# MrSwordFish/rvel-mcmc

Measured on AMD Instinct MI355X. Metric: walker-logL evals/sec (2-planet, 100 obs, 4096 walkers); ESS/sec, higher is better.
Workload: dtype f64

## Files before the change

### include/rvmcmc.h

```cpp
#ifndef RVMCMC_H
#define RVMCMC_H

#include <stddef.h>
#include <stdint.h>

#ifdef __cplusplus
extern "C" {
#endif

#define RVM_ABI_VERSION 12

#define RVM_STATUS_OK 0
#define RVM_STATUS_PRIOR 1
#define RVM_STATUS_ENCOUNTER 2
#define RVM_STATUS_NONFINITE 3
#define RVM_STATUS_UNRESOLVED 4
#define RVM_STATUS_SKIPPED 5

#define RVM_MAX_PLANETS 4
#define RVM_MAX_LEVELS 6
#define RVM_MAX_EPOCHS_PER_DIRECTION 1700
#define RVM_SMALA_MAX_PARAMS 20
#define RVM_RESOLVE_MAX_LIMIT 12

// ... 8 lines not shown
    double resolve_tol;
    int32_t resolve_max;
} rvm_config;

typedef struct rvm_plan rvm_plan;

int rvm_plan_create(const rvm_config* cfg, const double* t, const double* rv, const double* sigma, int32_t n_obs,
                    int32_t max_walkers, rvm_plan** out);
void rvm_plan_destroy(rvm_plan* plan);
int rvm_plan_info(const rvm_plan* plan, int32_t* steps_fwd, int32_t* steps_bwd, int32_t* epochs_fwd,
                  int32_t* epochs_bwd);
#define RVM_EXT_MAX_BYTES (4ull << 30)
int rvm_plan_extension(const rvm_plan* plan, int32_t* ext_mult);
int rvm_plan_set_verify_eccentricity(rvm_plan* plan, double e);

int rvm_plan_set_certain_reject(rvm_plan* plan, int32_t on);

int rvm_plan_faults(rvm_plan* plan, int32_t reset, int64_t* handoff_timeouts, int64_t* nonfinite,
                    int64_t* unresolved, int64_t* refined, int64_t* truncated, void* stream);
#define RVM_N_COUNTERS 7
int rvm_plan_counters(rvm_plan* plan, int32_t reset, int64_t* out, int32_t n, void* stream);
int rvm_plan_hedge_stats(rvm_plan* plan, int32_t reset, int64_t* hedged, int64_t* replayed, int64_t* missed,
                         void* stream);
int rvm_plan_time_kernels(rvm_plan* plan, int32_t max_launches);
int rvm_plan_kernel_times(rvm_plan* plan, float* logl_ms, float* refine_ms, int32_t max, int32_t* n_out);
int rvm_plan_set_handoff_timeout(rvm_plan* plan, double seconds);

int rvm_logl_batch(const rvm_plan* plan, int32_t n_walkers, const double* params, double hill_factor,
                   double* logl_out, int32_t* status_out, double* rv_out, void* stream);


int rvm_stretch_propose(int32_t n_params, int32_t n_s0, int64_t s0_begin, const double* x, int32_t n_s1,
                        const double* c, double a, uint64_t seed, uint64_t iteration, uint32_t half,
                        const double* draws, double* q_out, double* z_out, void* stream);
int rvm_stretch_accept(int32_t n_params, int32_t n_s0, int64_t s0_begin, double* x, double* lnp, const double* q,
                       const double* lnp_new, const double* z, uint64_t seed, uint64_t iteration, uint32_t half,
                       const double* draws, int32_t* accepted, void* stream);

#define RVM_MAX_PARAM_ROWS (7 * RVM_MAX_PLANETS)
typedef struct rvm_param_map {
    int32_t n_rows;
    int32_t src[RVM_MAX_PARAM_ROWS];
    double base[RVM_MAX_PARAM_ROWS];
} rvm_param_map;

int rvm_stretch_half_step(const rvm_plan* plan, const rvm_param_map* map, int32_t n_params, int32_t n_s0,
// ... 106 lines not shown
```

### rvel-mcmc_amd/csrc/host_sanitize.cpp

```cpp
#include <cmath>
#include <cstdio>
#include <cstring>
#include <vector>

#include "../../include/rvmcmc.h"

int main() {
    int fails = 0;
    auto expect = [&](bool ok, const char* what) {
        if (!ok) {
            std::fprintf(stderr, "FAIL %s\n", what);
            fails++;
        }
    };
    expect(rvm_abi_version() == RVM_ABI_VERSION, "abi version");
    rvm_config cfg{};
    cfg.n_planets = 2;
    cfg.dt = 0.65;
    cfg.n_levels = 4;
    cfg.npoints_norm = 100.0;
    const int mult[4] = {4, 5, 6, 7};
    std::memcpy(cfg.level_mult, mult, sizeof(mult));
    cfg.period_hint = 5.2;
    std::vector<double> t, rv, sg;
// ... 1 lines not shown
        t.push_back(i % 2 ? -0.6 * i : 0.55 * (100 - i));
        rv.push_back(1e-4 * std::sin(i));
        sg.push_back(1.5e-4);
    }
    t[7] = t[9];
    rvm_plan* plan = nullptr;
    const int rc = rvm_plan_create(&cfg, t.data(), rv.data(), sg.data(), (int)t.size(), 4096, &plan);
    expect(rc == 0 || (rc < 0 && plan == nullptr), "plan_create valid input");
    if (rc == 0) rvm_plan_destroy(plan);
    rvm_config bad = cfg;
    bad.n_levels = 0;
    expect(rvm_plan_create(&bad, t.data(), rv.data(), sg.data(), (int)t.size(), 64, &plan) < 0, "n_levels 0");
    bad = cfg;
    bad.level_mult[1] = 4;
    expect(rvm_plan_create(&bad, t.data(), rv.data(), sg.data(), (int)t.size(), 64, &plan) < 0, "dup multipliers");
    bad = cfg;
    bad.dt = -1.0;
    expect(rvm_plan_create(&bad, t.data(), rv.data(), sg.data(), (int)t.size(), 64, &plan) < 0, "negative dt");
    std::vector<double> tn = t;
    tn[3] = NAN;
    expect(rvm_plan_create(&cfg, tn.data(), rv.data(), sg.data(), (int)t.size(), 64, &plan) < 0, "nan epoch");
    expect(std::strlen(rvm_last_error()) > 0, "last_error");
    expect(rvm_logl_batch(nullptr, 1, nullptr, 1.0, nullptr, nullptr, nullptr, nullptr) < 0, "logl null plan");
    rvm_param_map pm{};
    expect(rvm_stretch_half_step(nullptr, &pm, 10, 1, 0, nullptr, nullptr, nullptr, 1, nullptr, 2.0, 0, 0, 0, 1.0,
                                 nullptr, nullptr, nullptr, nullptr) < 0,
           "half_step null plan");
    expect(rvm_stretch_propose(0, 1, 0, nullptr, 1, nullptr, 2.0, 0, 0, 0, nullptr, nullptr, nullptr, nullptr) < 0,
           "propose bad");
    double d1 = 0.5;
    int32_t i1 = 0;
    expect(rvm_pt_stretch_propose(10, 0, 1, &d1, &d1, 2.0, 0, 0, 0, nullptr, &d1, &d1, nullptr) < 0, "pt n_temps 0");
    expect(rvm_pt_stretch_propose(10, 2, 1, &d1, &d1, 1.0, 0, 0, 0, nullptr, &d1, &d1, nullptr) < 0, "pt a = 1");
    expect(rvm_pt_stretch_propose(10, 1 << 16, 1 << 16, &d1, &d1, 2.0, 0, 0, 0, nullptr, &d1, &d1, nullptr) < 0,
           "pt int32 overflow");
    expect(rvm_pt_stretch_accept(10, 2, 1, nullptr, &d1, &d1, &d1, &d1, &d1, 0, 0, 0, nullptr, &i1, nullptr) < 0,
           "pt null betas");
    expect(rvm_pt_stretch_accept(10, 2, 1, &d1, &d1, &d1, &d1, &d1, &d1, 0, 0, 2, nullptr, &i1, nullptr) < 0,
           "pt half 2");
    expect(rvm_pt_swap(10, 2, 0, &d1, &d1, &d1, &d1, &d1, 0, 0, nullptr, &i1, nullptr) < 0, "pt n_half 0");
    expect(rvm_pt_swap(10, 1 << 15, 1 << 15, &d1, &d1, &d1, &d1, &d1, 0, 0, nullptr, &i1, nullptr) < 0,
           "pt swap int32 overflow");
    expect(rvm_pt_swap(10, 1, 4, nullptr, nullptr, nullptr, nullptr, nullptr, 0, 0, nullptr, nullptr, nullptr) == 0,
           "pt swap of one temperature");
    int64_t l1 = 0;
    expect(rvm_pt_ladder_update(3, 1, &i1, &d1, &d1, -1.0, &d1, &l1, &d1, &l1, nullptr, &d1, nullptr) < 0,
// ... 20 lines not shown
```

### rvel-mcmc_amd/csrc/rvm_abi.hip

```cpp
#include <hip/hip_runtime.h>

#include <algorithm>
#include <cmath>
#include <cstdio>
#include <cstdlib>
#include <cstring>
#include <string>
#include <vector>

#include "rvm_internal.h"

#ifndef RVM_EAGER_DEFAULT
#define RVM_EAGER_DEFAULT true
#endif
#ifndef RVM_EAGER_PASSES_DEFAULT
#define RVM_EAGER_PASSES_DEFAULT 1
#endif

namespace rvm {
hipError_t launch_logl(const DevPlan& P, int W, const double* params, double hill_factor, unsigned long long* slots,
                       double* logl, int32_t* status, double* rv_out, const StretchArgs& sa, hipStream_t stream,
                       int* dry_blocks);
hipError_t launch_refine(const DevPlan& P, int W, const double* params, double hill_factor, double* logl,
                         int32_t* status, double* rv_out, const StretchArgs& sa, int eager, int hedge,
// ... 492 lines not shown
        P.rq_tf = reinterpret_cast<unsigned long long*>(base + b_x + b_xf + b_t);
        P.rq_c = reinterpret_cast<double*>(base + b_x + b_xf + b_t + b_tf);
        P.rq_w = reinterpret_cast<int32_t*>(base + b_x + b_xf + b_t + b_tf + b_c);
        P.rq_n = reinterpret_cast<int32_t*>(base + b_x + b_xf + b_t + b_tf + b_c + b_w);
        P.gen_dev = reinterpret_cast<unsigned long long*>(base + b_x + b_xf + b_t + b_tf + b_c + b_w + 32);
        P.depth_w = reinterpret_cast<unsigned long long*>(base + b_x + b_xf + b_t + b_tf + b_c + b_w + 64 + b_m);
        P.rq_mark = reinterpret_cast<int32_t*>(base + b_x + b_xf + b_t + b_tf + b_c + b_w + 64);
        const unsigned long long gen1 = 1;
        if (hipMemcpy(P.gen_dev, &gen1, sizeof(gen1), hipMemcpyHostToDevice) != hipSuccess) {
            (void)hipGetLastError();
            rvm_plan_destroy(plan);
            return fail(-3, "rvm_plan_create: initialising the launch generation failed");
        }
        P.rq_cap = max_walkers;
        P.rq_xgroups = (int32_t)xg;
        if (const char* sp = getenv("RVM_REFINE_SPLIT"))
            if (sp[0] == '0') P.rq_x = nullptr;
        if (n_teams < 2) P.rq_t = nullptr;
        if (const char* th = getenv("RVM_TEAMS_HINT"))
            if (th[0] == '0') P.depth_w = nullptr;
        P.n_teams = (int32_t)nt;
    }
    P.hedge_groups = 0;
    P.hrv = nullptr;
    P.hsum = nullptr;
    P.hslot = nullptr;
    P.htab = nullptr;
    P.hw = nullptr;
    {
        const char* eg = getenv("RVM_EAGER");
        const bool eager_on = eg ? eg[0] == '1' : RVM_EAGER_DEFAULT;
        const int emw = std::min<int>(max_walkers, rvm::RVM_EAGER_MAX);
        const char* hg = getenv("RVM_HEDGE");
        int hgroups = hg && hg[0] == '0' ? 0 : rvm::RVM_HEDGE_GROUPS_MAX;
        if (const char* hn = getenv("RVM_HEDGE_GROUPS"))
            hgroups = std::min(hgroups, std::max(0, std::min(atoi(hn), (int)rvm::RVM_HEDGE_GROUPS_MAX)));
        if (hgroups > 0 && P.rmax >= 2 && P.rvp != nullptr && P.gen_dev != nullptr && cfg->n_levels <= 4 &&
            max_walkers >= rvm::RVM_EAGER_MIN && P.n_cu >= 4) {
            const size_t hs = rvm::RVM_HEDGE_STRIDE;
            const size_t n_rv = 2 * (size_t)P.lvx_emax * hs, n_sum = 6 * hs, n_slot = 2 * hs;
            const size_t n_all = n_rv + n_sum + n_slot + (size_t)max_walkers + rvm::RVM_HW_WORDS;
            if (hipMalloc(&plan->hmem, n_all * sizeof(double)) == hipSuccess &&
                hipMemset(plan->hmem, 0, n_all * sizeof(double)) == hipSuccess && hipDeviceSynchronize() == hipSuccess) {
                P.hrv = reinterpret_cast<double*>(plan->hmem);
                P.hsum = P.hrv + n_rv;
                P.hslot = reinterpret_cast<unsigned long long*>(P.hsum + n_sum);
                P.htab = P.hslot + n_slot;
                P.hw = P.htab + max_walkers;
                P.hedge_groups = hgroups;
            } else {
                (void)hipGetLastError();
                if (plan->hmem) (void)hipFree(plan->hmem);
                plan->hmem = nullptr;
            }
        }
        const bool eager_plan = P.rmax >= 2 && P.rvp != nullptr && P.gen_dev != nullptr && cfg->n_levels <= 4 &&
                                eager_on && max_walkers >= rvm::RVM_EAGER_MIN;
        if (!eager_plan && P.hedge_groups > 0) {
            if (hipStreamCreateWithFlags(&plan->side, hipStreamNonBlocking) != hipSuccess ||
                hipEventCreateWithFlags(&plan->ev_fork, hipEventDisableTiming) != hipSuccess ||
                hipEventCreateWithFlags(&plan->ev_join, hipEventDisableTiming) != hipSuccess) {
                (void)hipGetLastError();
                if (plan->ev_fork) (void)hipEventDestroy(plan->ev_fork);
                if (plan->ev_join) (void)hipEventDestroy(plan->ev_join);
                if (plan->side) (void)hipStreamDestroy(plan->side);
                plan->side = nullptr;
                plan->ev_fork = plan->ev_join = nullptr;
                P.hedge_groups = 0;
            }
        }
        if (eager_plan) {
            const size_t plane = (size_t)P.lvx_emax * P.lvx_stride;
// ... 97 lines not shown
        if (plan->lvmem) e = hipMemsetAsync(plan->lvmem, 0xFF, plan->lv_bytes, st);
        if (e == hipSuccess) e = hipMemsetAsync(plan->dev.counters, 0, sizeof(h), st);
        if (e == hipSuccess) e = hipStreamSynchronize(st);
        if (e != hipSuccess) return hip_fail(e, "rvm_plan_counters: reset");
    }
    return 0;
}

int rvm_plan_hedge_stats(rvm_plan* plan, int32_t reset, int64_t* hedged, int64_t* replayed, int64_t* missed,
                         void* stream) {
    if (!plan) return fail(-1, "rvm_plan_hedge_stats: null plan");
    unsigned long long h[3] = {};
    if (plan->dev.hw != nullptr) {
        hipStream_t st = (hipStream_t)stream;
        unsigned long long* d = plan->dev.hw + rvm::RVM_HW_STATS;
        hipError_t e = hipMemcpyAsync(h, d, sizeof(h), hipMemcpyDeviceToHost, st);
        if (e == hipSuccess && reset) e = hipMemsetAsync(d, 0, sizeof(h), st);
        if (e == hipSuccess) e = hipStreamSynchronize(st);
        if (e != hipSuccess) return hip_fail(e, "rvm_plan_hedge_stats");
    }
    if (hedged) *hedged = (int64_t)h[0];
    if (replayed) *replayed = (int64_t)h[1];
    if (missed) *missed = (int64_t)h[2];
    return 0;
}

int rvm_plan_faults(rvm_plan* plan, int32_t reset, int64_t* handoff_timeouts, int64_t* nonfinite,
                    int64_t* unresolved, int64_t* refined, int64_t* truncated, void* stream) {
    if (!plan) return fail(-1, "rvm_plan_faults: null plan");
    int64_t c[RVM_N_COUNTERS] = {};
    const int rc = rvm_plan_counters(plan, reset, c, RVM_N_COUNTERS, stream);
    if (rc != 0) return rc;
    if (handoff_timeouts) *handoff_timeouts = c[0];
    if (nonfinite) *nonfinite = c[1];
    if (unresolved) *unresolved = c[2];
    if (refined) *refined = c[3];
    if (truncated) *truncated = c[4];
    return 0;
}

int rvm_plan_time_kernels(rvm_plan* plan, int32_t max_launches) {
    if (!plan) return fail(-1, "rvm_plan_time_kernels: null plan");
    if (max_launches < 0 || max_launches > 4096) return fail(-1, "rvm_plan_time_kernels: max_launches out of range");
    while ((int32_t)plan->tev.size() < 3 * max_launches) {
        hipEvent_t ev;
        const hipError_t e = hipEventCreate(&ev);
// ... 527 lines not shown
```

### rvel-mcmc_amd/csrc/rvm_internal.h

```cpp
#pragma once
#include <stdint.h>

#include "../../include/rvmcmc.h"

namespace rvm {

constexpr int RVM_LS_RING = 64;
constexpr int RVM_LC_RING = 16;
constexpr int RVM_LC_RING_BYTES = 24 * 1024;
constexpr int RVM_LDS_PER_CU = 160 * 1024;
constexpr int RVM_INIT_DOUBLES = 8 * 64;
constexpr double RVM_EXT_ACCEPT = 1.0;
constexpr double RVM_CUT_EST_FACTOR = 100.0;
constexpr double RVM_FLOOR_BOUND = 4.0;
constexpr double RVM_CUT_ECC_FACTOR = 0.6712;
constexpr double RVM_CUT_GUARD_K = 10.0;
constexpr int RVM_CX_MIN_WALKERS = 32;
constexpr int RVM_EAGER_MAX = 512;
constexpr int RVM_EAGER_MIN = 32;
constexpr int RVM_EFLAG_WORDS = 8;
constexpr int RVM_TEAMS_MAX = 4;
constexpr int RVM_TEAMS_DEFAULT = 4;
constexpr int RVM_DEPTH_WINDOW = 8;
constexpr int RVM_HEDGE_GROUPS_MAX = 8;
constexpr int RVM_HEDGE_STRIDE = 512;
constexpr int RVM_HEDGE_CAND = RVM_HEDGE_STRIDE + 64;
constexpr int RVM_HEDGE_MAX_W = 12288;
constexpr int RVM_HW_STATS = 2 + 2 * RVM_HEDGE_GROUPS_MAX;
constexpr int RVM_HW_WORDS = RVM_HW_STATS + 3 + 3;

struct DirSched {
    int32_t n_epochs;
    int32_t n_steps;
    int32_t split0, pre0, split1, pre1;
    const int32_t* seg_n;
    const double* seg_h1;
    const double* obs_rv;
    const double* obs_s2;
    const int32_t* obs_idx;
};

struct DevPlan {
    int32_t n_planets;
    int32_t n_levels;
    int32_t mult[RVM_MAX_LEVELS];
    int32_t nt[RVM_MAX_LEVELS];
    int32_t spec[RVM_MAX_LEVELS];
    int32_t late_mult;
    int32_t lc_ring;
    double inv_mult[RVM_MAX_LEVELS];
    double lw[RVM_MAX_LEVELS];
    double lw3[RVM_MAX_LEVELS];
// ... 11 lines not shown
    double cut_guard_k;
    int32_t lvx_emax, lvx_stride;
    int32_t* rq_n;
    int32_t* rq_w;
    double* rq_c;
    int32_t rq_cap;
    int32_t* rq_mark;
    int32_t skip_variants;
    unsigned long long* rq_x;
    unsigned long long* rq_xf;
    int32_t rq_xgroups;
    unsigned long long* rq_t;
    unsigned long long* rq_tf;
    double* rvp2;
    int32_t n_teams;
    unsigned long long* depth_w;
    double* rve;
    double* esum;
    unsigned long long* eflag;
    int32_t eager_max;
    int32_t eager_passes;
    int32_t eager_split;
    int32_t hedge_groups;
    double* hrv;
    double* hsum;
    unsigned long long* hslot;
    unsigned long long* htab;
    unsigned long long* hw;
    unsigned long long* gen_dev;
    unsigned long long* counters;
    unsigned long long spin_ticks;
    double npoints;
    int32_t n_obs;
    int32_t inclined;
    int32_t n_cu;
    double* lv_rv;
    int32_t* lv_enc;
    int32_t lv_emax, lv_stride;
    DirSched fwd, bwd;
};

struct StretchArgs {
    const double* c;
    double* x;
    double* x_aos;
    double* lnp;
// ... 71 lines not shown
```

### rvel-mcmc_amd/csrc/rvm_refine_impl.h

```cpp
#pragma once
#include <hip/hip_runtime.h>
#include <math.h>

#pragma clang fp contract(on)

#include "rvm_walker.h"

#ifndef RVM_REFINE_GUESS
#define RVM_REFINE_GUESS 0
#endif
#ifndef RVM_REFINE_RELAXED_COUNT
#define RVM_REFINE_RELAXED_COUNT 0
#endif

namespace rvm {

#ifdef RVM_PROFILE
#define RVM_RPROF_SLOTS 20
#define RVM_RPROF_MAX_WAVES 4096
static __device__ unsigned long long rvm_rprof[RVM_RPROF_MAX_WAVES * RVM_RPROF_SLOTS];
#define RPROF_T(v) const unsigned long long v = __builtin_readcyclecounter()
#define RPROF_RT(v) const unsigned long long v = __builtin_amdgcn_s_memrealtime()
#else
#define RPROF_T(v)
#define RPROF_RT(v)
#endif

__device__ __forceinline__ bool claim_item(gu64* w, unsigned long long gen, unsigned long long code) {
    unsigned long long v = __hip_atomic_load(w, __ATOMIC_RELAXED, __HIP_MEMORY_SCOPE_AGENT);
    for (;;) {
        if ((v >> 8) == gen) return false;
        unsigned long long expect = v;
        if (__hip_atomic_compare_exchange_strong(w, &expect, (gen << 8) | code, __ATOMIC_RELAXED, __ATOMIC_RELAXED,
                                                 __HIP_MEMORY_SCOPE_AGENT))
            return true;
        v = expect;
    }
}

__device__ __forceinline__ unsigned long long pass_ticks(const DevPlan& P, int rf) {
    const unsigned long long t = P.spin_ticks << (rf < RVM_RESOLVE_MAX_LIMIT ? rf : RVM_RESOLVE_MAX_LIMIT);
    constexpr unsigned long long cap = 6000000000ull;
    return t < cap ? t : (P.spin_ticks > cap ? P.spin_ticks : cap);
}

struct DirState {
    int open;
    double chi, lb, pest, best, bchi;
};

template <int NP, bool D3, int NW>
__global__ __launch_bounds__(NW * 64) void refine_kernel(const DevPlan P, const int W, const double* __restrict__ params,
                                                     const double hill_factor, double* __restrict__ rv_out,
                                                     double* __restrict__ logl_out, int32_t* __restrict__ status_out,
                                                     const StretchArgs sa, const int eager, const int hedge) {
    constexpr int L = LanesPerWalker<NP>::value;
    constexpr int WPB = 64 / L;
    constexpr int PR = D3 ? 7 : 5;
    constexpr int R = PR * NP;
    const int wv = threadIdx.x >> 6;
    const int lane = threadIdx.x & 63;
    const int slot = lane / L;
    const int pl_idx = lane % L;
    const int nl = P.n_levels;
    RPROF_T(pt_entry);
    RPROF_RT(prt_entry);
#ifdef RVM_PROFILE
    unsigned long long p_seg = 0, p_epo = 0, p_steps = 0, p_wait = 0, p_pass = 0;
    int p_lvl = -1;
#endif

    __shared__ int s_n[3];
    __shared__ unsigned long long s_gen;
    __shared__ int s_depth;
    if (threadIdx.x == 0) {
        for (int i = 0; i < 3; i++) s_n[i] = __hip_atomic_load(P.rq_n + i, __ATOMIC_RELAXED, __HIP_MEMORY_SCOPE_AGENT);
        const unsigned long long g0 = __hip_atomic_load(P.gen_dev, __ATOMIC_RELAXED, __HIP_MEMORY_SCOPE_AGENT);
        s_gen = g0;
// ... 35 lines not shown
            gu64* hw = (gu64*)P.hw;
            if (__hip_atomic_fetch_add(hw + 1, 1ull, __ATOMIC_RELAXED, __HIP_MEMORY_SCOPE_AGENT) + 1 == gridDim.x) {
                __hip_atomic_store(hw + 1, 0ull, __ATOMIC_RELAXED, __HIP_MEMORY_SCOPE_AGENT);
                __hip_atomic_store(hw, (gen << 8) | 1ull, __ATOMIC_RELAXED, __HIP_MEMORY_SCOPE_AGENT);
            }
        }
    };
    const bool split = !eager && P.rq_x != nullptr && gq0 <= P.rq_xgroups && ((int)gridDim.x & 1) == 0 &&
                       ntask_split <= gfit;
    int nteam = 0;
    if (split && P.rq_t != nullptr && P.rvp != nullptr && P.rvp2 != nullptr && rv_out == nullptr &&
        ng <= P.rq_xgroups) {
        nteam = P.n_teams < P.rmax ? P.n_teams : P.rmax;
        if (nteam > (depth_hint > 2 ? depth_hint : 2)) nteam = depth_hint > 2 ? depth_hint : 2;
        while (nteam >= 2 && nteam * ntask_split > gfit) nteam--;
    }
    const bool team = nteam >= 2;
    const int ntask_team = nteam * ntask_split;
    const int ngw = (W + WPB - 1) / WPB;
    const bool esplit = eager && P.eager_split && P.rq_x != nullptr && ngw <= P.rq_xgroups &&
                        ((int)gridDim.x & 1) == 0 && 2 * ngw <= (int)gridDim.x;
    const int ntask = eager ? (esplit ? 2 * ngw : ngw) : (team ? ntask_team : (split ? ntask_split : ng));
    if ((int)blockIdx.x >= ntask) {
        leave();
        return;
    }

    extern __shared__ double s_sched[];
    __shared__ double s_rv[2][2][RVM_MAX_LEVELS][64];
    __shared__ int s_enc[2][RVM_MAX_LEVELS][64];
    __shared__ double s_init[8][64];
    __shared__ double s_chi[2][64], s_lb[2][64];
    __shared__ double s_pest[2][64], s_best[2][64], s_bchi[2][64];
    __shared__ int s_open[2][64];
    __shared__ int s_live[64];
    __shared__ int s_stw[64];
    __shared__ double s_lpw[64];
    __shared__ double s_acc[3][64];
    __shared__ int s_dmode[64];
    __shared__ unsigned long long s_mask[2];
    __shared__ int s_xfault;
    __shared__ double s_tc2[2][64], s_te2[2][64];
    __shared__ int s_ter[2][64];
    __shared__ int s_cancel[2];
    __shared__ int s_eitems[64], s_eli[64], s_eany;
    __shared__ int s_emask;
// ... 965 lines not shown
    const int pl_idx = lane % L;
    const int nl = P.n_levels;
    const int g = blockIdx.x >> 1, dd = blockIdx.x & 1;
    const DirSched& SR = dd ? P.bwd : P.fwd;
    const int Er = SR.n_epochs;
    extern __shared__ unsigned long long s_key[];
    __shared__ double s_rv[2][RVM_MAX_LEVELS][64];
    __shared__ int s_enc[RVM_MAX_LEVELS][64];
    __shared__ int s_cnt[2][256];
    __shared__ unsigned long long s_ck[RVM_HEDGE_CAND];
    __shared__ int s_ci[RVM_HEDGE_CAND];
    __shared__ int s_sel[64];
    __shared__ int s_cancel[2];
    __shared__ unsigned long long s_gen, s_pref;
    __shared__ int s_need;
#ifdef RVM_PROFILE
    const unsigned long long prt_entry = __builtin_amdgcn_s_memrealtime();
#endif
    gu64* hw = (gu64*)P.hw;
    if (tid == 0) s_gen = __hip_atomic_load(P.gen_dev, __ATOMIC_RELAXED, __HIP_MEMORY_SCOPE_AGENT);
    __syncthreads();
    const unsigned long long gen = s_gen;
    const unsigned long long ctag = (gen << 8) | 1ull;
    if (tid == 0) s_cancel[0] = __hip_atomic_load(hw, __ATOMIC_RELAXED, __HIP_MEMORY_SCOPE_AGENT) == ctag;
    __syncthreads();
    if (s_cancel[0]) return;
    const unsigned long long kbad = ~0ull;
    for (int i = tid; i < RVM_HEDGE_CAND; i += 256) {
        s_ck[i] = kbad;
        s_ci[i] = 0;
    }
    for (int i = tid; i < W; i += 256) {
        int kind = 0, wk = i, jst = 0, jp = 0;
        double zst = 0.0, zp = 0.0;
        stretch_slot(sa, i, kind, wk, zst, jst, zp, jp);
        double sc = INFINITY;
        bool ok = true;
#pragma unroll
        for (int p = 0; p < NP; p++) {
            const double m = walker_param(true, nullptr, W, wk, sa, PR * p + 0, zst, jst, kind, zp, jp);
            const double a = walker_param(true, nullptr, W, wk, sa, PR * p + 1, zst, jst, kind, zp, jp);
            const double h = walker_param(true, nullptr, W, wk, sa, PR * p + 2, zst, jst, kind, zp, jp);
            const double k = walker_param(true, nullptr, W, wk, sa, PR * p + 3, zst, jst, kind, zp, jp);
            const double e = sqrt(h * h + k * k);
            ok = ok && a > 0.02 && m > 5e-6 && e < 1.0;
            sc = fmin(sc, a * (1.0 - e) / cbrt(1.0 + m));
        }
        ok = ok && isfinite(sc) && sc > 0.0;
        s_key[i] = ok ? (unsigned long long)__double_as_longlong(sc) : kbad;
// ... 135 lines not shown
    KickPrep<NP> kq0{};
    if (work && Er > 0) kq0 = kick_prep<NP, L, D3>(s, 1.875);
    constexpr int rf = 2;
    const int m_r = P.mult[k_u] << rf;
    const int nt_r = P.nt[k_u];
    const bool late = P.late_mult > 0 && m_r >= P.late_mult;
    const double sc = ldexp(P.inv_mult[k_u], -rf);
    const bool cmb = work && k == 0 && lane < cnt;
    const int hx = g * WPB + (cmb ? lane : 0);
    gu64* rvo = (gu64*)(P.hrv + (size_t)dd * P.lvx_emax * RVM_HEDGE_STRIDE + hx);
    double c2 = 0.0, e2 = 0.0;
    bool cancelled = false;
#ifdef RVM_PROFILE
    const unsigned long long prt_loop0 = __builtin_amdgcn_s_memrealtime();
#endif
    for (int e = 0; e < Er; e++) {
        const int ns = __builtin_amdgcn_readfirstlane(work ? SR.seg_n[e] * m_r : 0);
        if (ns > 0)
            (void)segment_gated_c<D3, NP, L, RVM_REFINE_GUESS>(s, kq0, SR.seg_h1[e] * sc, ns, nt_r, hw, nullptr, ctag, late);
        if (work) {
            const double v0 = star_vx<NP, L>(s);
            if (pl_idx == 0) s_rv[e & 1][k_u][slot] = v0;
        }
        if (wv == 0 && lane == 0)
            s_cancel[e & 1] = __hip_atomic_load(hw, __ATOMIC_RELAXED, __HIP_MEMORY_SCOPE_AGENT) == ctag;
        __syncthreads();
        if (s_cancel[e & 1]) {
            cancelled = true;
            break;
        }
        if (cmb) {
            double rvx = 0.0, rv3 = 0.0;
            for (int q = 0; q < nl; q++) rvx += P.lw[q] * s_rv[e & 1][q][lane];
            for (int q = 1; q < nl; q++) rv3 += P.lw3[q] * s_rv[e & 1][q][lane];
            const double ob = SR.obs_rv[e], s2 = SR.obs_s2[e];
            const double r = rvx - ob;
            c2 += (r * r) / s2;
            e2 += fabs((rvx - rv3) * (r + (rv3 - ob))) / s2;
            __hip_atomic_store(rvo + (size_t)e * RVM_HEDGE_STRIDE, (unsigned long long)__double_as_longlong(rvx),
                               __ATOMIC_RELAXED, __HIP_MEMORY_SCOPE_AGENT);
        }
    }
#ifdef RVM_PROFILE
    if (lane == 0 && RVM_RPROF_MAX_WAVES / 2 + (size_t)blockIdx.x * 8 + wv < RVM_RPROF_MAX_WAVES) {
        unsigned long long* o = rvm_rprof + (RVM_RPROF_MAX_WAVES / 2 + (size_t)blockIdx.x * 8 + wv) * RVM_RPROF_SLOTS;
        o[0] = prt_entry;
        o[1] = prt_loop0;
        o[2] = __builtin_amdgcn_s_memrealtime();
        o[3] = o[2];
        o[9] = (unsigned long long)blockIdx.x | (1ull << 29) | ((unsigned long long)(cancelled ? 1 : 0) << 30);
        o[10] = cancelled ? 0 : 1;
        o[11] = (unsigned long long)(unsigned)__builtin_amdgcn_s_getreg((31 << 11) | 4);
    }
#endif
    if (cancelled) return;
    if (work && pl_idx == 0) s_enc[k_u][slot] = (int)(((s.encm >> lane) & kick_enc_bits<NP>()) != 0);
    __syncthreads();
    if (wv == 0) {
        if (__builtin_amdgcn_readfirstlane((int)(__hip_atomic_load(hw, __ATOMIC_RELAXED, __HIP_MEMORY_SCOPE_AGENT) == ctag)))
            return;
        if (cmb) {
            int er = 0;
            for (int q = 0; q < nl; q++) er |= s_enc[q][lane];
            gu64* es = (gu64*)(P.hsum + (size_t)dd * 3 * RVM_HEDGE_STRIDE + hx);
            auto bits = [](double v) { return (unsigned long long)__double_as_longlong(v); };
            __hip_atomic_store(es, bits(c2), __ATOMIC_RELAXED, __HIP_MEMORY_SCOPE_AGENT);
            __hip_atomic_store(es + RVM_HEDGE_STRIDE, bits(e2), __ATOMIC_RELAXED, __HIP_MEMORY_SCOPE_AGENT);
            __hip_atomic_store(es + 2 * RVM_HEDGE_STRIDE, bits((double)er), __ATOMIC_RELAXED, __HIP_MEMORY_SCOPE_AGENT);
        }
        asm volatile("s_waitcnt vmcnt(0)" ::: "memory");
        if (lane == 0)
            __hip_atomic_store(hw + 2 + 2 * g + dd, (gen << 8) | 2ull, __ATOMIC_RELAXED, __HIP_MEMORY_SCOPE_AGENT);
    }
}

template <int NPV, bool D3V>
static size_t hedge_budget() {
    static size_t budget[64] = {};
    static bool known[64] = {};
    int dev = 0;
    if (hipGetDevice(&dev) != hipSuccess || dev < 0 || dev >= 64) {
        (void)hipGetLastError();
        return 0;
// ... 52 lines not shown
        }
        (void)hipGetLastError();
        budget[dev] = b;
    }
    return budget[dev];
}

template <int NPV, bool D3V>
static hipError_t launch_refine_t(const DevPlan& P, int W, const double* params, double hill_factor, double* logl,
                                  int32_t* status, double* rv_out, const StretchArgs& sa, int eager, int hedge,
                                  hipStream_t stream) {
    constexpr int wpb = 64 / LanesPerWalker<NPV>::value;
    const int emax = P.fwd.n_epochs > P.bwd.n_epochs ? P.fwd.n_epochs : P.bwd.n_epochs;
    const size_t smem = (size_t)emax * 8 * sizeof(double);
    static const bool w4_env = [] {
        const char* e = getenv("RVM_REFINE_W4");
        return !(e && e[0] == '0');
    }();
    const bool w4 = P.n_levels <= 4 && w4_env;
    if (smem > (w4 ? refine_budget<NPV, D3V, 4>() : refine_budget<NPV, D3V, 8>())) return hipErrorInvalidConfiguration;
    const int groups = (W + wpb - 1) / wpb + 2;
    int nb = std::max(2, std::min(P.n_cu > 0 ? P.n_cu : 256, 2 * groups));
    nb &= ~1;
    if (w4)
        refine_kernel<NPV, D3V, 4><<<dim3(nb), dim3(256), smem, stream>>>(P, W, params, hill_factor, rv_out, logl, status,
                                                                          sa, eager, hedge);
    else
        refine_kernel<NPV, D3V, 8><<<dim3(nb), dim3(512), smem, stream>>>(P, W, params, hill_factor, rv_out, logl, status,
                                                                          sa, eager, hedge);
    return hipGetLastError();
}

template <int NPV, bool D3V>
static hipError_t prepare_refine_t(const DevPlan& P) {
    const int emax = P.fwd.n_epochs > P.bwd.n_epochs ? P.fwd.n_epochs : P.bwd.n_epochs;
    const size_t smem = (size_t)emax * 8 * sizeof(double);
    const size_t b = std::min(refine_budget<NPV, D3V, 4>(), refine_budget<NPV, D3V, 8>());
    if (P.hedge_groups > 0) (void)hedge_budget<NPV, D3V>();
    return smem <= b ? hipSuccess : hipErrorInvalidConfiguration;
}

#define RVM_REFINE_NP_API(N)                                                                                     \
    hipError_t launch_refine_np##N(const DevPlan& P, int W, const double* params, double hill_factor, double* logl, \
                                   int32_t* status, double* rv_out, const StretchArgs& sa, int eager, int hedge, \
                                   hipStream_t stream);                                                          \
    int hedge_groups_np##N(const DevPlan& P, int W, int logl_blocks);                                           \
    hipError_t launch_hedge_np##N(const DevPlan& P, int W, double hill_factor, const StretchArgs& sa, int ngrp, \
                                  hipStream_t stream);                                                           \
    hipError_t launch_eager_np##N(const DevPlan& P, int W, const double* params, double hill_factor,            \
                                  hipStream_t stream);                                                           \
    hipError_t prepare_refine_np##N(const DevPlan& P);
RVM_REFINE_NP_API(1)
RVM_REFINE_NP_API(2)
RVM_REFINE_NP_API(3)
RVM_REFINE_NP_API(4)
#undef RVM_REFINE_NP_API

}
```

### rvel-mcmc_amd/rvmcmc/_lib.py

```python
from __future__ import annotations

import ctypes as C
import os

_HERE = os.path.dirname(os.path.abspath(__file__))
LIB_PATH = os.environ.get("RVM_LIB_PATH") or os.path.join(_HERE, "librvmcmc.so")

RVM_STATUS_OK = 0
RVM_STATUS_PRIOR = 1
RVM_STATUS_ENCOUNTER = 2
RVM_STATUS_NONFINITE = 3
RVM_STATUS_UNRESOLVED = 4
RVM_STATUS_SKIPPED = 5
RVM_MAX_PLANETS = 4
RVM_MAX_LEVELS = 6
RVM_N_COUNTERS = 7
ABI_VERSION = 12


class RvmConfig(C.Structure):
    _fields_ = [
        ("n_planets", C.c_int32),
        ("dt", C.c_double),
        ("n_levels", C.c_int32),
# ... 46 lines not shown
                                         C.c_double, C.c_double, C.c_double, C.POINTER(SmalaCache), _dp]),
    "rvm_smala_center_accept": (C.c_int, [C.c_int32, C.c_int32, C.c_int64, _dp, _dp, _dp, _dp, C.POINTER(SmalaCache),
                                          C.POINTER(SmalaCache), C.c_double, C.c_uint64, C.c_uint64, _dp, _dp, _dp,
                                          _dp]),
    "rvm_smala_metric_accept": (C.c_int, [C.c_int32, C.c_int32, C.c_int64, _dp, _dp, _dp, _dp, _dp, _dp, C.c_double,
                                          C.c_double, C.POINTER(SmalaCache), C.POINTER(SmalaCache), C.c_uint64,
                                          C.c_uint64, _dp, _dp, _dp, _dp]),
    "rvm_last_error": (C.c_char_p, []),
    "rvm_plan_create": (C.c_int, [C.POINTER(RvmConfig), C.POINTER(C.c_double), C.POINTER(C.c_double),
                                  C.POINTER(C.c_double), C.c_int32, C.c_int32, C.POINTER(C.c_void_p)]),
    "rvm_plan_destroy": (None, [C.c_void_p]),
    "rvm_plan_faults": (C.c_int, [C.c_void_p, C.c_int32, C.POINTER(C.c_int64), C.POINTER(C.c_int64),
                                  C.POINTER(C.c_int64), C.POINTER(C.c_int64), C.POINTER(C.c_int64), _dp]),
    "rvm_plan_set_handoff_timeout": (C.c_int, [C.c_void_p, C.c_double]),
    "rvm_plan_time_kernels": (C.c_int, [C.c_void_p, C.c_int32]),
    "rvm_plan_kernel_times": (C.c_int, [C.c_void_p, C.POINTER(C.c_float), C.POINTER(C.c_float), C.c_int32,
                                        C.POINTER(C.c_int32)]),
    "rvm_plan_extension": (C.c_int, [C.c_void_p, C.POINTER(C.c_int32)]),
    "rvm_plan_set_verify_eccentricity": (C.c_int, [C.c_void_p, C.c_double]),
    "rvm_plan_set_certain_reject": (C.c_int, [C.c_void_p, C.c_int32]),
    "rvm_plan_counters": (C.c_int, [C.c_void_p, C.c_int32, C.POINTER(C.c_int64), C.c_int32, C.c_void_p]),
    "rvm_plan_hedge_stats": (C.c_int, [C.c_void_p, C.c_int32, C.POINTER(C.c_int64), C.POINTER(C.c_int64),
                                       C.POINTER(C.c_int64), C.c_void_p]),
    "rvm_plan_info": (C.c_int, [C.c_void_p, C.POINTER(C.c_int32), C.POINTER(C.c_int32), C.POINTER(C.c_int32),
                                C.POINTER(C.c_int32)]),
    "rvm_logl_batch": (C.c_int, [C.c_void_p, C.c_int32, _dp, C.c_double, _dp, _dp, _dp, _dp]),
    "rvm_stretch_propose": (C.c_int, [C.c_int32, C.c_int32, C.c_int64, _dp, C.c_int32, _dp, C.c_double, C.c_uint64,
                                      C.c_uint64, C.c_uint32, _dp, _dp, _dp, _dp]),
    "rvm_stretch_accept": (C.c_int, [C.c_int32, C.c_int32, C.c_int64, _dp, _dp, _dp, _dp, _dp, C.c_uint64, C.c_uint64,
                                     C.c_uint32, _dp, _dp, _dp]),
    "rvm_pt_stretch_propose": (C.c_int, [C.c_int32, C.c_int32, C.c_int32, _dp, _dp, C.c_double, C.c_uint64,
                                         C.c_uint64, C.c_uint32, _dp, _dp, _dp, _dp]),
    "rvm_pt_stretch_accept": (C.c_int, [C.c_int32, C.c_int32, C.c_int32, _dp, _dp, _dp, _dp, _dp, _dp, C.c_uint64,
                                        C.c_uint64, C.c_uint32, _dp, _dp, _dp]),
    "rvm_pt_swap": (C.c_int, [C.c_int32, C.c_int32, C.c_int32, _dp, _dp, _dp, _dp, _dp, C.c_uint64, C.c_uint64, _dp,
                              _dp, _dp]),
    "rvm_pt_ladder_update": (C.c_int, [C.c_int32, C.c_int32, _dp, _dp, _dp, C.c_double, _dp, _dp, _dp, _dp, _dp, _dp,
                                       _dp]),
    "rvm_stretch_half_step": (C.c_int, [C.c_void_p, C.POINTER(ParamMapC), C.c_int32, C.c_int32, C.c_int64, _dp, _dp,
                                        _dp, C.c_int32, _dp, C.c_double, C.c_uint64, C.c_uint64, C.c_uint32,
                                        C.c_double, _dp, _dp, _dp, _dp]),
    "rvm_stretch_iteration_begin": (C.c_int, [C.c_void_p, C.POINTER(ParamMapC), C.c_int32, C.c_int32, C.c_int64,
                                              C.c_int64, _dp, _dp, _dp, _dp, C.c_int32, _dp, _dp, C.c_double, C.c_uint64,
                                              C.c_uint64, C.c_double, _dp, _dp, _dp, _dp, _dp]),
    "rvm_stretch_iteration_end": (C.c_int, [C.c_int32, C.c_int32, C.c_int64, C.c_int64, _dp, _dp, _dp, _dp, _dp,
                                            _dp, _dp, C.c_int32, _dp, _dp, _dp, _dp, C.c_double, C.c_uint64,
# ... 50 lines not shown
```

### rvel-mcmc_amd/rvmcmc/engine.py

```python
from __future__ import annotations

import ctypes as C
import math
from dataclasses import dataclass
from typing import Optional

import numpy as np

from . import _lib

KERNEL_KEYS = ("m", "a", "h", "k", "l")
KERNEL_KEYS_INCLINED = KERNEL_KEYS + ("ix", "iy")
SUPPORTED_KEYS = set(KERNEL_KEYS_INCLINED)


def level_multipliers(levels) -> tuple:
    if isinstance(levels, (int, np.integer)):
        mult = tuple(range(1, int(levels) + 1))
    else:
        mult = tuple(int(m) for m in levels)
    if not 1 <= len(mult) <= _lib.RVM_MAX_LEVELS:
        raise ValueError(f"1..{_lib.RVM_MAX_LEVELS} Richardson levels supported, got {len(mult)}")
    if len(set(mult)) != len(mult) or min(mult) < 1 or max(mult) > 64:
        raise ValueError("level multipliers must be distinct integers in 1..64")
# ... 121 lines not shown
            _lib.check(self.lib.rvm_plan_set_verify_eccentricity(self._h, self.ecc_guard),
                       "rvm_plan_set_verify_eccentricity")
        if not self.certain_reject:
            _lib.check(self.lib.rvm_plan_set_certain_reject(self._h, 0), "rvm_plan_set_certain_reject")

    def faults(self, reset=False, stream=None) -> dict:
        vals = (C.c_int64 * _lib.RVM_N_COUNTERS)()
        _lib.check(self.lib.rvm_plan_counters(self._h, int(bool(reset)), vals, _lib.RVM_N_COUNTERS,
                                              _lib.stream_handle(stream)), "rvm_plan_counters")
        f = dict(handoff_timeouts=vals[0], nonfinite=vals[1], unresolved=vals[2], refined=vals[3],
                 truncated=vals[4], floor_settled=vals[5], skipped=vals[6])
        if reset:
            tot = self.__dict__.setdefault("totals", dict.fromkeys(f, 0))
            for k, v in f.items():
                tot[k] += v
        return f

    def hedge_stats(self, reset=False, stream=None) -> dict:
        h, r, m = C.c_int64(), C.c_int64(), C.c_int64()
        _lib.check(self.lib.rvm_plan_hedge_stats(self._h, int(bool(reset)), C.byref(h), C.byref(r), C.byref(m),
                                                 _lib.stream_handle(stream)), "rvm_plan_hedge_stats")
        return dict(hedged=h.value, replayed=r.value, missed=m.value)

    def check_faults(self, what="plan", stream=None, group=None) -> dict:
        f = self.faults(reset=True, stream=stream)
        bad = [f["handoff_timeouts"], f["nonfinite"], f["unresolved"] if self.resolve_max > 0 else 0]
        if group is not None:
            torch = _torch()
            dist = torch.distributed
            dev = self.device if dist.get_backend(group) == "nccl" else torch.device("cpu")
            t = torch.tensor(bad, dtype=torch.int64, device=dev)
            dist.all_reduce(t, group=group)
            bad = [int(v) for v in t.cpu()]
        if any(bad):
            raise _lib.RvmError(f"{what}: {bad[0]} level-split hand-off timeout(s), {bad[1]} non-finite "
                                f"log-likelihood(s), {bad[2]} walker(s) not resolved to the plan's tolerance after "
                                f"{self.resolve_max} halvings on the GPU (rvm_plan_faults"
                                f"{', summed over the ranks' if group is not None else ''})")
        return f

    def time_kernels(self, max_launches):
        _lib.check(self.lib.rvm_plan_time_kernels(self._h, int(max_launches)), "rvm_plan_time_kernels")

    def kernel_times(self, max_launches=4096):
        a = (C.c_float * max_launches)()
        b = (C.c_float * max_launches)()
# ... 266 lines not shown
```

Baseline: 3.076 million.

## Mark hedge groups with no pending refine work so hedge blocks stop early

Adds a refine-kernel variant in which an idle trailing block scans the refine queues and flags hedge groups whose walkers no longer need speculative hedged integration. Hedge blocks poll these per-group marks alongside the global cancel tag and exit early, which frees compute units otherwise spent on redundant hedge work. The behaviour is on by default whenever hedging is active (it can be disabled with RVM_HEDGE_MARK=0), and counters plus a new ABI query report how many groups were marked or abandoned. The cost is an extra atomic load per poll, plus the risk of marking a group too early if the queue snapshot is stale.

```diff
diff --git a/include/rvmcmc.h b/include/rvmcmc.h
--- a/include/rvmcmc.h
+++ b/include/rvmcmc.h
@@ -54,6 +54,7 @@
 int rvm_plan_counters(rvm_plan* plan, int32_t reset, int64_t* out, int32_t n, void* stream);
 int rvm_plan_hedge_stats(rvm_plan* plan, int32_t reset, int64_t* hedged, int64_t* replayed, int64_t* missed,
                          void* stream);
+int rvm_plan_hedge_marks(rvm_plan* plan, int32_t reset, int64_t* marked, int64_t* gave_up, void* stream);
 int rvm_plan_time_kernels(rvm_plan* plan, int32_t max_launches);
 int rvm_plan_kernel_times(rvm_plan* plan, float* logl_ms, float* refine_ms, int32_t max, int32_t* n_out);
 int rvm_plan_set_handoff_timeout(rvm_plan* plan, double seconds);
diff --git a/rvel-mcmc_amd/csrc/host_sanitize.cpp b/rvel-mcmc_amd/csrc/host_sanitize.cpp
--- a/rvel-mcmc_amd/csrc/host_sanitize.cpp
+++ b/rvel-mcmc_amd/csrc/host_sanitize.cpp
@@ -47,6 +47,8 @@
     expect(rvm_plan_create(&cfg, tn.data(), rv.data(), sg.data(), (int)t.size(), 64, &plan) < 0, "nan epoch");
     expect(std::strlen(rvm_last_error()) > 0, "last_error");
     expect(rvm_logl_batch(nullptr, 1, nullptr, 1.0, nullptr, nullptr, nullptr, nullptr) < 0, "logl null plan");
+    int64_t mk = -1, gu = -1;
+    expect(rvm_plan_hedge_marks(nullptr, 0, &mk, &gu, nullptr) < 0 && mk == -1 && gu == -1, "hedge_marks null plan");
     rvm_param_map pm{};
     expect(rvm_stretch_half_step(nullptr, &pm, 10, 1, 0, nullptr, nullptr, nullptr, 1, nullptr, 2.0, 0, 0, 0, 1.0,
                                  nullptr, nullptr, nullptr, nullptr) < 0,
diff --git a/rvel-mcmc_amd/csrc/rvm_abi.hip b/rvel-mcmc_amd/csrc/rvm_abi.hip
--- a/rvel-mcmc_amd/csrc/rvm_abi.hip
+++ b/rvel-mcmc_amd/csrc/rvm_abi.hip
@@ -538,6 +538,7 @@
         P.n_teams = (int32_t)nt;
     }
     P.hedge_groups = 0;
+    P.hedge_mark = 0;
     P.hrv = nullptr;
     P.hsum = nullptr;
     P.hslot = nullptr;
@@ -564,6 +565,8 @@
                 P.htab = P.hslot + n_slot;
                 P.hw = P.htab + max_walkers;
                 P.hedge_groups = hgroups;
+                const char* hm = getenv("RVM_HEDGE_MARK");
+                P.hedge_mark = hm && hm[0] == '0' ? 0 : 1;
             } else {
                 (void)hipGetLastError();
                 if (plan->hmem) (void)hipFree(plan->hmem);
@@ -707,6 +710,22 @@
     if (hedged) *hedged = (int64_t)h[0];
     if (replayed) *replayed = (int64_t)h[1];
     if (missed) *missed = (int64_t)h[2];
+    return 0;
+}
+
+int rvm_plan_hedge_marks(rvm_plan* plan, int32_t reset, int64_t* marked, int64_t* gave_up, void* stream) {
+    if (!plan) return fail(-1, "rvm_plan_hedge_marks: null plan");
+    unsigned long long h[2] = {};
+    if (plan->dev.hw != nullptr) {
+        hipStream_t st = (hipStream_t)stream;
+        unsigned long long* d = plan->dev.hw + rvm::RVM_HW_STATS + 3;
+        hipError_t e = hipMemcpyAsync(h, d, sizeof(h), hipMemcpyDeviceToHost, st);
+        if (e == hipSuccess && reset) e = hipMemsetAsync(d, 0, sizeof(h), st);
+        if (e == hipSuccess) e = hipStreamSynchronize(st);
+        if (e != hipSuccess) return hip_fail(e, "rvm_plan_hedge_marks");
+    }
+    if (marked) *marked = (int64_t)h[0];
+    if (gave_up) *gave_up = (int64_t)h[1];
     return 0;
 }
 
diff --git a/rvel-mcmc_amd/csrc/rvm_internal.h b/rvel-mcmc_amd/csrc/rvm_internal.h
--- a/rvel-mcmc_amd/csrc/rvm_internal.h
+++ b/rvel-mcmc_amd/csrc/rvm_internal.h
@@ -27,7 +27,8 @@
 constexpr int RVM_HEDGE_CAND = RVM_HEDGE_STRIDE + 64;
 constexpr int RVM_HEDGE_MAX_W = 12288;
 constexpr int RVM_HW_STATS = 2 + 2 * RVM_HEDGE_GROUPS_MAX;
-constexpr int RVM_HW_WORDS = RVM_HW_STATS + 3 + 3;
+constexpr int RVM_HW_MARK = RVM_HW_STATS + 3 + 3;
+constexpr int RVM_HW_WORDS = RVM_HW_MARK + 2 * RVM_HEDGE_GROUPS_MAX;
 
 struct DirSched {
     int32_t n_epochs;
@@ -85,6 +86,7 @@
     int32_t eager_passes;
     int32_t eager_split;
     int32_t hedge_groups;
+    int32_t hedge_mark;
     double* hrv;
     double* hsum;
     unsigned long long* hslot;
diff --git a/rvel-mcmc_amd/csrc/rvm_refine_impl.h b/rvel-mcmc_amd/csrc/rvm_refine_impl.h
--- a/rvel-mcmc_amd/csrc/rvm_refine_impl.h
+++ b/rvel-mcmc_amd/csrc/rvm_refine_impl.h
@@ -38,6 +38,34 @@
     }
 }
 
+__device__ __forceinline__ void hedge_mark_unneeded(const int32_t* rq_w, const int rq_cap,
+                                                    const unsigned long long* htab, unsigned long long* hw_,
+                                                    const int n0, const int n1, const int n2,
+                                                    const unsigned long long gen, const int hedge, const int wpb) {
+    const int lane = threadIdx.x & 63;
+    unsigned need = 0;
+    for (int l2 = 0; l2 < 3; l2++) {
+        int n = l2 == 0 ? n0 : (l2 == 1 ? n1 : n2);
+        n = n < rq_cap ? n : rq_cap;
+        for (int i = lane; i < n; i += 64) {
+            const int wl = rq_w[(size_t)l2 * rq_cap + i];
+            if (wl < 0 || wl >= rq_cap) continue;
+            const unsigned long long tb = __hip_atomic_load((gu64*)htab + wl, __ATOMIC_RELAXED, __HIP_MEMORY_SCOPE_AGENT);
+            const int hg = (int)(tb & 0xFFFF) / wpb;
+            if ((tb >> 16) != gen || hg >= RVM_HEDGE_GROUPS_MAX) continue;
+            if (l2 != 2) need |= 1u << (2 * hg);
+            if (l2 != 1) need |= 1u << (2 * hg + 1);
+        }
+    }
+    for (int d = 32; d >= 1; d >>= 1) need |= (unsigned)__shfl_xor((int)need, d, 64);
+    gu64* hw = (gu64*)hw_;
+    const bool mark = lane < hedge && lane < 2 * RVM_HEDGE_GROUPS_MAX && !((need >> lane) & 1u);
+    if (mark) __hip_atomic_store(hw + RVM_HW_MARK + lane, (gen << 8) | 1ull, __ATOMIC_RELAXED, __HIP_MEMORY_SCOPE_AGENT);
+    const unsigned long long nm = __builtin_popcountll(ballot(mark));
+    if (lane == 0 && nm)
+        __hip_atomic_fetch_add(hw + RVM_HW_STATS + 3, nm, __ATOMIC_RELAXED, __HIP_MEMORY_SCOPE_AGENT);
+}
+
 __device__ __forceinline__ unsigned long long pass_ticks(const DevPlan& P, int rf) {
     const unsigned long long t = P.spin_ticks << (rf < RVM_RESOLVE_MAX_LIMIT ? rf : RVM_RESOLVE_MAX_LIMIT);
     constexpr unsigned long long cap = 6000000000ull;
@@ -49,11 +77,13 @@
     double chi, lb, pest, best, bchi;
 };
 
+constexpr int RVM_REFINE_HM = 5;
 template <int NP, bool D3, int NW>
-__global__ __launch_bounds__(NW * 64) void refine_kernel(const DevPlan P, const int W, const double* __restrict__ params,
-                                                     const double hill_factor, double* __restrict__ rv_out,
-                                                     double* __restrict__ logl_out, int32_t* __restrict__ status_out,
-                                                     const StretchArgs sa, const int eager, const int hedge) {
+__global__ __launch_bounds__((NW == RVM_REFINE_HM ? 4 : NW) * 64) void refine_kernel(
+    const DevPlan P, const int W, const double* __restrict__ params, const double hill_factor,
+    double* __restrict__ rv_out, double* __restrict__ logl_out, int32_t* __restrict__ status_out, const StretchArgs sa,
+    const int eager, const int hedge) {
+    constexpr bool HM = NW == RVM_REFINE_HM;
     constexpr int L = LanesPerWalker<NP>::value;
     constexpr int WPB = 64 / L;
     constexpr int PR = D3 ? 7 : 5;
@@ -135,6 +165,10 @@
                         ((int)gridDim.x & 1) == 0 && 2 * ngw <= (int)gridDim.x;
     const int ntask = eager ? (esplit ? 2 * ngw : ngw) : (team ? ntask_team : (split ? ntask_split : ng));
     if ((int)blockIdx.x >= ntask) {
+        if constexpr (HM) {
+            if (hedge && blockIdx.x == gridDim.x - 1 && wv == 0)
+                hedge_mark_unneeded(P.rq_w, P.rq_cap, P.htab, P.hw, nq[0], nq[1], nq[2], gen, hedge, WPB);
+        }
         leave();
         return;
     }
@@ -1146,9 +1180,25 @@
     __syncthreads();
     const unsigned long long gen = s_gen;
     const unsigned long long ctag = (gen << 8) | 1ull;
-    if (tid == 0) s_cancel[0] = __hip_atomic_load(hw, __ATOMIC_RELAXED, __HIP_MEMORY_SCOPE_AGENT) == ctag;
+    __shared__ int s_marked;
+    auto stopped = [&]() {
+        const bool mk = __hip_atomic_load(hw + RVM_HW_MARK + blockIdx.x, __ATOMIC_RELAXED, __HIP_MEMORY_SCOPE_AGENT) == ctag;
+        if (mk) s_marked = 1;
+        return mk || __hip_atomic_load(hw, __ATOMIC_RELAXED, __HIP_MEMORY_SCOPE_AGENT) == ctag;
+    };
+    if (tid == 0) {
+        s_marked = 0;
+        s_cancel[0] = stopped();
+    }
     __syncthreads();
-    if (s_cancel[0]) return;
+    auto count_marked = [&]() {
+        if (tid == 0 && s_marked)
+            __hip_atomic_fetch_add(hw + RVM_HW_STATS + 4, 1ull, __ATOMIC_RELAXED, __HIP_MEMORY_SCOPE_AGENT);
+    };
+    if (s_cancel[0]) {
+        count_marked();
+        return;
+    }
     const unsigned long long kbad = ~0ull;
     for (int i = tid; i < RVM_HEDGE_CAND; i += 256) {
         s_ck[i] = kbad;
@@ -1330,8 +1380,7 @@
             const double v0 = star_vx<NP, L>(s);
             if (pl_idx == 0) s_rv[e & 1][k_u][slot] = v0;
         }
-        if (wv == 0 && lane == 0)
-            s_cancel[e & 1] = __hip_atomic_load(hw, __ATOMIC_RELAXED, __HIP_MEMORY_SCOPE_AGENT) == ctag;
+        if (wv == 0 && lane == 0) s_cancel[e & 1] = stopped();
         __syncthreads();
         if (s_cancel[e & 1]) {
             cancelled = true;
@@ -1361,12 +1410,17 @@
         o[11] = (unsigned long long)(unsigned)__builtin_amdgcn_s_getreg((31 << 11) | 4);
     }
 #endif
-    if (cancelled) return;
+    if (cancelled) {
+        count_marked();
+        return;
+    }
     if (work && pl_idx == 0) s_enc[k_u][slot] = (int)(((s.encm >> lane) & kick_enc_bits<NP>()) != 0);
     __syncthreads();
     if (wv == 0) {
-        if (__builtin_amdgcn_readfirstlane((int)(__hip_atomic_load(hw, __ATOMIC_RELAXED, __HIP_MEMORY_SCOPE_AGENT) == ctag)))
+        if (__builtin_amdgcn_readfirstlane((int)stopped())) {
+            count_marked();
             return;
+        }
         if (cmb) {
             int er = 0;
             for (int q = 0; q < nl; q++) er |= s_enc[q][lane];
@@ -1465,7 +1519,10 @@
     const int groups = (W + wpb - 1) / wpb + 2;
     int nb = std::max(2, std::min(P.n_cu > 0 ? P.n_cu : 256, 2 * groups));
     nb &= ~1;
-    if (w4)
+    if (w4 && hedge && P.hedge_mark && smem <= refine_budget<NPV, D3V, RVM_REFINE_HM>())
+        refine_kernel<NPV, D3V, RVM_REFINE_HM><<<dim3(nb), dim3(256), smem, stream>>>(P, W, params, hill_factor, rv_out,
+                                                                                      logl, status, sa, eager, hedge);
+    else if (w4)
         refine_kernel<NPV, D3V, 4><<<dim3(nb), dim3(256), smem, stream>>>(P, W, params, hill_factor, rv_out, logl, status,
                                                                           sa, eager, hedge);
     else
@@ -1480,6 +1537,7 @@
     const size_t smem = (size_t)emax * 8 * sizeof(double);
     const size_t b = std::min(refine_budget<NPV, D3V, 4>(), refine_budget<NPV, D3V, 8>());
     if (P.hedge_groups > 0) (void)hedge_budget<NPV, D3V>();
+    if (P.hedge_groups > 0 && P.hedge_mark) (void)refine_budget<NPV, D3V, RVM_REFINE_HM>();
     return smem <= b ? hipSuccess : hipErrorInvalidConfiguration;
 }
 
diff --git a/rvel-mcmc_amd/rvmcmc/_lib.py b/rvel-mcmc_amd/rvmcmc/_lib.py
--- a/rvel-mcmc_amd/rvmcmc/_lib.py
+++ b/rvel-mcmc_amd/rvmcmc/_lib.py
@@ -92,6 +92,7 @@
     "rvm_plan_counters": (C.c_int, [C.c_void_p, C.c_int32, C.POINTER(C.c_int64), C.c_int32, C.c_void_p]),
     "rvm_plan_hedge_stats": (C.c_int, [C.c_void_p, C.c_int32, C.POINTER(C.c_int64), C.POINTER(C.c_int64),
                                        C.POINTER(C.c_int64), C.c_void_p]),
+    "rvm_plan_hedge_marks": (C.c_int, [C.c_void_p, C.c_int32, C.POINTER(C.c_int64), C.POINTER(C.c_int64), C.c_void_p]),
     "rvm_plan_info": (C.c_int, [C.c_void_p, C.POINTER(C.c_int32), C.POINTER(C.c_int32), C.POINTER(C.c_int32),
                                 C.POINTER(C.c_int32)]),
     "rvm_logl_batch": (C.c_int, [C.c_void_p, C.c_int32, _dp, C.c_double, _dp, _dp, _dp, _dp]),
diff --git a/rvel-mcmc_amd/rvmcmc/engine.py b/rvel-mcmc_amd/rvmcmc/engine.py
--- a/rvel-mcmc_amd/rvmcmc/engine.py
+++ b/rvel-mcmc_amd/rvmcmc/engine.py
@@ -167,6 +167,12 @@
                                                  _lib.stream_handle(stream)), "rvm_plan_hedge_stats")
         return dict(hedged=h.value, replayed=r.value, missed=m.value)
 
+    def hedge_marks(self, reset=False, stream=None) -> dict:
+        m, g = C.c_int64(), C.c_int64()
+        _lib.check(self.lib.rvm_plan_hedge_marks(self._h, int(bool(reset)), C.byref(m), C.byref(g),
+                                                 _lib.stream_handle(stream)), "rvm_plan_hedge_marks")
+        return dict(marked=m.value, gave_up=g.value)
+
     def check_faults(self, what="plan", stream=None, group=None) -> dict:
         f = self.faults(reset=True, stream=stream)
         bad = [f["handoff_timeouts"], f["nonfinite"], f["unresolved"] if self.resolve_max > 0 else 0]
```

New measurement: 3.152 million (median of 6 runs). 1.02x the previous value.
